# votnhan/VN_celeb_face_recognition

Hardware: AMD Instinct MI355X
Metric: embeddings/sec @ bs=256 (InceptionResnetV1, 160x160) (higher is better)
Workload: dtype bf16

## Files before the change

vn_celeb_face_recognition_amd/csrc/engine.h:

```cpp
#pragma once
#include <hip/hip_runtime.h>
#include <stdint.h>

#include <string>
#include <unordered_map>
#include <vector>

#include "../../include/vnface.h"
#include "kernels.h"

namespace vnf {

void set_error(const std::string& msg);
int fail(int code, const std::string& msg);
const char* last_error_cstr();

#define VNF_HIP(expr)                                                                         \
  do {                                                                                        \
    hipError_t _e = (expr);                                                                   \
    if (_e != hipSuccess)                                                                     \
      return ::vnf::fail(VNF_E_HIP, std::string(#expr) + ": " + hipGetErrorString(_e));       \
  } while (0)

enum class HandleKind { Encoder = 1, Mlp, Mtcnn, MlpTrainer, Retina, HeadTrainer, ConvProbe, Gallery };

struct HandleBase {
  const HandleKind kind;
  explicit HandleBase(HandleKind k) : kind(k) {}
  int device = 0;
  std::vector<void*> allocs;
  virtual ~HandleBase();
  void* dalloc(size_t bytes);
  void* upload(const void* host, size_t bytes);
};

template <class T>
T* handle_cast(vnf_handle h) {
  HandleBase* b = reinterpret_cast<HandleBase*>(h);
  return (b && b->kind == T::KIND) ? static_cast<T*>(b) : nullptr;
}

template <class T>
T* handle_cast_base(vnf_handle h) {
  HandleBase* b = reinterpret_cast<HandleBase*>(h);
  if (b)
    for (HandleKind k : T::KINDS)
      if (b->kind == k) return static_cast<T*>(b);
  return nullptr;
}

struct WeightMap {
  std::unordered_map<std::string, const vnf_tensor_desc*> m;
  std::string missing;
  WeightMap(const vnf_tensor_desc* w, int n);
  const float* get(const std::string& name, int64_t numel);
  bool has(const std::string& name) const { return m.count(name) != 0; }
};

void convert_to(int dtype, const float* src, void* dst, size_t n);

struct Buf {
  int H, W, C;
  size_t elems_per_image() const { return (size_t)H * W * C; }
  char* ptr = nullptr;
};

struct ConvLayer {
  std::string name;
  int x_buf, x_coff, cin;
  int H, W, Ho, Wo, KH, KW, sh, sw, ph, pw;
  void* w = nullptr;
  float* bias = nullptr;
  float* slope = nullptr;
  int4* ktab = nullptr;
  int K, Kpad, cout, cout_pad, ncls = 1;
  int nseg = 0;
  struct { int c0, c1, buf, coff; } seg[4];
  int res_buf = -1, res_coff = 0;
  int act = ACT_NONE, out_f32 = 0;
  int cfg = -1;
  double macs_alg = 0, macs_exec = 0;
};

struct Op {
  enum Kind { PACK, CONV, MAXPOOL, AVGPOOL, L2NORM, COPYOUT, STEM1, DWCONV, UPADD, RSTEM, DWPW, HEADS, SE } kind;
  int src = -1;
  int dst = -1, dst_coff = 0;
  int layer = -1;
  int res = -1;
  PoolWindow window = {0, 0, false};
  int frame_h = 0, frame_w = 0;
  int n_cls = 0, n_proj = 0, proj_col = 0;

  static Op pack(int dst) { Op o{PACK}; o.dst = dst; return o; }
  static Op conv(int layer) { Op o{CONV}; o.layer = layer; return o; }
  static Op stem1(int layer, int dst) { Op o{STEM1}; o.layer = layer; o.dst = dst; return o; }
  static Op maxpool(int src, int dst, int dst_coff, PoolWindow w = {3, 0, false}) {
    Op o{MAXPOOL}; o.src = src; o.dst = dst; o.dst_coff = dst_coff; o.window = w; return o;
  }
  static Op maxpool_ceil(int src, int dst, int k) { return maxpool(src, dst, 0, {k, 0, true}); }
  static Op maxpool_pad1(int src, int dst) { return maxpool(src, dst, 0, {3, 1, false}); }
  static Op avgpool(int src, int dst) { Op o{AVGPOOL}; o.src = src; o.dst = dst; return o; }
  static Op l2norm() { return Op{L2NORM}; }
  static Op copyout() { return Op{COPYOUT}; }
  static Op dwconv(int layer) { Op o{DWCONV}; o.layer = layer; return o; }
  static Op dwpw(int layer) { Op o{DWPW}; o.layer = layer; return o; }
  static Op upadd(int src, int dst) { Op o{UPADD}; o.src = src; o.dst = dst; return o; }
  static Op rstem(int frame_h, int frame_w, int dst) { Op o{RSTEM}; o.frame_h = frame_h; o.frame_w = frame_w; o.dst = dst; return o; }
  static Op se(int layer, int src, int res, int dst) { Op o{SE}; o.layer = layer; o.src = src; o.res = res; o.dst = dst; return o; }
  static Op heads(int n_cls, int n_proj, int proj_col) { Op o{HEADS}; o.n_cls = n_cls; o.n_proj = n_proj; o.proj_col = proj_col; return o; }
};

struct DwLayer {
  int x_buf, o_buf, C, stride;
  float *w = nullptr, *bias = nullptr;
  float slope = 0.f;
};

struct DwPwLayer {
  int x_buf, o_buf, cin, cout, stride;
  float *dw = nullptr, *dbias = nullptr, *pw = nullptr, *pbias = nullptr;
  float slope = 0.f;
  std::string name;
};

struct SeLayer {
  std::string name;
  int C, part_buf;
  float *w1 = nullptr, *b1 = nullptr, *w2 = nullptr, *b2 = nullptr;
  float slope_se = 0.f, slope_out = 0.f;
};

struct Group { int first, last, chunk; };

struct FusedStack {
  enum class Kind { StemMid, Block35, Block17, Block8 } kind = Kind::Block17;
  std::string label;
  int first = 0, last = 0;
  int in_buf = -1, out_buf = -1;
  int nblocks = 0;
  int conv0 = 0;
  void* wstream = nullptr;
  float* bias = nullptr;
  void* wtail = nullptr;
  bool active = false;
  bool stack = false;
  double macs_alg = 0;
  int ext_last = 0, ext_conv = -1, ext_out_buf = -1;
  bool ext = false;
  int end() const { return ext ? ext_last : last; }
};

struct Tap { int buf, coff, C; };

struct EncoderEnv {
  int fuse = 95, direct_stem = 1, stem1a_mfma = 2, retina_fuse = 3, ws_persist = 1;
  int stem_chunk = 0, ir100_chunk1 = 0, ir100_chunk2 = 0;
  int autotune = 1, force_cfg = -2, tune_lanes = 0, autotune_log = 0;
  bool tune_final = true;
  std::string tune_cache;
  static EncoderEnv read();
};

struct RunExtra {
  float* out2 = nullptr;
  const uint8_t* prep_src = nullptr;
  int prep_s = 0;
};

constexpr int ARCH_MLP = -1, ARCH_RNET = -2, ARCH_ONET = -3, ARCH_RETINA = -5;

struct Encoder : HandleBase {
  static constexpr HandleKind KIND = HandleKind::Encoder;
  Encoder() : HandleBase(KIND) {}
  ~Encoder() override;
  int arch, dtype, max_batch, in_size;
  std::vector<Buf> bufs;
  std::vector<ConvLayer> convs;
  std::vector<DwLayer> dws;
  std::vector<DwPwLayer> dwpws;
  std::vector<SeLayer> ses;
  float *rstem_wa = nullptr, *rstem_bias = nullptr;
  std::vector<Op> ops;
  std::vector<Group> groups;
  std::vector<FusedStack> fused;
  std::vector<int> fused_at;
  int prepare_fused();
  int launch_fused(const FusedStack& f, int n0, int nn, hipStream_t s);
  std::unordered_map<std::string, Tap> taps;
  bool buf_materialised(int buf) const;
  float* emb_raw = nullptr;
  int emb_ld = 512;
  int n_cls = 0, n_proj = 0;
  float* cls_buf = nullptr;
  double macs_alg = 0, macs_exec = 0;
  Encoder* head = nullptr;
  int head_classes = 0, head_in = -1, head_logit = -1;
  float* head_emb = nullptr;
  hipEvent_t head_done = nullptr;

  int add_buf(int H, int W, int C);
  char* at(int buf, int n0, int coff = 0) const {
    return bufs[buf].ptr + ((size_t)n0 * bufs[buf].elems_per_image() + coff) * dtype_size(dtype);
  }
  float* at_f32(int buf, int n0) const { return (float*)at(buf, n0); }
  int finalize();
  int autotune();
  ConvArgs conv_args(const ConvLayer& L, int n0, int nn) const;
  int run(const void* x, int n, int x_dtype, float* out, hipStream_t s, std::string* report = nullptr,
          const RunExtra* extra = nullptr);
  int run_range(const void* x, int i0, int i1, int x_dtype, float* out, hipStream_t s, std::string* report, const RunExtra* extra);
  int write_report(std::vector<hipEvent_t>& prof_ev, const std::vector<int>& prof_op, int n, hipStream_t s, std::string* report) const;
  float* stem_wt = nullptr;
  int n_ctx = 1, next_ctx = 0;
  std::vector<std::vector<char*>> ctx_bufs;
  std::vector<float*> ctx_emb;
  std::vector<hipEvent_t> ctx_ev;
  int select_ctx(hipStream_t s, int* used);
  int max_streams = 4;
  bool tune_dirty = true;
  int tune_lanes = 1;
  int tune_batch = 0;
  const EncoderEnv env = EncoderEnv::read();
  hipStream_t side[4] = {nullptr, nullptr, nullptr, nullptr};
  hipEvent_t join_ev[4] = {nullptr, nullptr, nullptr, nullptr}, fork_ev = nullptr;
};

const char* fused_label(const FusedStack& f);
const char* fused_detail(const FusedStack& f);

int build_irv1(Encoder& e, WeightMap& wm);
int build_ir100(Encoder& e, WeightMap& wm);
int build_seir101(Encoder& e, WeightMap& wm);
int build_rn50_2b(Encoder& e, WeightMap& wm, int num_classes, int num_projections);
int build_retina_mnet(Encoder& e, WeightMap& wm, int H, int W, int head_bufs[3]);
struct NetBufs { int crops, pooled1, pooled2, heads; };
int build_rnet(Encoder& e, WeightMap& wm, bool mid, NetBufs& nb);
int build_onet(Encoder& e, WeightMap& wm, bool mid, NetBufs& nb);

}
```

vn_celeb_face_recognition_amd/csrc/fused.cpp:

```cpp
#include "engine.h"
#include "block35.h"
#include "block8.h"
#include "stem_mid.h"
#include "trunk17.h"

#include <cstring>

namespace vnf {

using Kind = FusedStack::Kind;

namespace {

hipError_t copy_bias(float* dst, const ConvLayer& L) { return hipMemcpy(dst, L.bias, (size_t)L.cout * 4, hipMemcpyDeviceToDevice); }

int prepare_stem_mid(Encoder& e, FusedStack& f) {
  if (!(e.env.fuse & 4)) return VNF_OK;
  const ConvLayer& c2a = e.convs[f.conv0];
  const ConvLayer& c2b = e.convs[f.conv0 + 1];
  if (c2a.cout != 32 || c2a.K != 288 || c2b.cout != 64 || c2b.K != 288 || c2a.ncls != 1 || c2b.ncls != 1)
    return fail(VNF_E_INVALID, "fused stem: unexpected layer shapes");
  bool ext_ok = false;
  if ((e.env.fuse & 8) && f.ext_conv >= 0) {
    const ConvLayer& c3b = e.convs[f.ext_conv];
    ext_ok = c3b.cout == 80 && c3b.K == 64 && c3b.KH == 1 && c3b.ncls == 1 && c3b.nseg == 1 && c3b.res_buf < 0 && c3b.act == ACT_RELU &&
             e.bufs[f.ext_out_buf].C == 80;
  }
  if (e.dtype == F16P && !ext_ok) return VNF_OK;
  StemMidPack pk;
  pk.w[0] = c2a.w; pk.kpad[0] = c2a.Kpad;
  pk.w[1] = c2b.w; pk.kpad[1] = c2b.Kpad;
  f.wstream = e.dalloc(stem_mid_wfrag_bytes(e.dtype));
  f.bias = (float*)e.dalloc(SM_BIAS * 4);
  if (!f.wstream || !f.bias) return VNF_E_HIP;
  VNF_HIP(copy_bias(f.bias, c2a));
  VNF_HIP(copy_bias(f.bias + 32, c2b));
  VNF_HIP(stem_mid_repack(pk, e.dtype, f.wstream, 0));
  VNF_HIP(hipDeviceSynchronize());
  f.macs_alg = c2a.macs_alg + c2b.macs_alg;
  f.active = true;
  f.ext = ext_ok;
  if (ext_ok) f.macs_alg += e.convs[f.ext_conv].macs_alg;
  return VNF_OK;
}

int prepare_block35(Encoder& e, FusedStack& f) {
  if (!(e.env.fuse & 2)) return VNF_OK;
  static const int rows[5] = {96, 32, 32, 32, 256}, ks[5] = {256, 288, 288, 288, 96}, boff[5] = {0, 96, 128, 160, 192};
  const size_t wimg_bytes = block35_wimg_bytes(e.dtype);
  f.wstream = e.dalloc((size_t)f.nblocks * wimg_bytes);
  f.bias = (float*)e.dalloc((size_t)f.nblocks * B35_BIAS * 4);
  if (!f.wstream || !f.bias) return VNF_E_HIP;
  for (int b = 0; b < f.nblocks; ++b) {
    Block35Pack pk;
    float* bias = f.bias + (size_t)b * B35_BIAS;
    pk.bias = bias;
    for (int c = 0; c < 5; ++c) {
      const ConvLayer& L = e.convs[f.conv0 + 5 * b + c];
      if (L.cout != rows[c] || L.K != ks[c] || L.ncls != 1) return fail(VNF_E_INVALID, "fused Block35: unexpected layer shapes");
      pk.w[c] = L.w;
      pk.kpad[c] = L.Kpad;
      VNF_HIP(copy_bias(bias + boff[c], L));
      f.macs_alg += L.macs_alg;
    }
    VNF_HIP(block35_repack(pk, e.dtype, (char*)f.wstream + (size_t)b * wimg_bytes, 0));
  }
  VNF_HIP(hipDeviceSynchronize());
  f.active = true;
  f.stack = (e.env.fuse & 16) && e.dtype != F16P;
  f.ext = false;
  if (f.stack && (e.env.fuse & 32) && f.ext_conv >= 0) {
    const ConvLayer& t = e.convs[f.ext_conv];
    const ConvLayer& last_up = e.convs[f.conv0 + 5 * (f.nblocks - 1) + 4];
    const bool ok = t.KH == 1 && t.KW == 1 && t.K == 256 && t.cout == 192 && t.ncls == 1 && t.nseg == 1 && t.res_buf < 0 &&
                    t.act == ACT_RELU && !t.out_f32 && t.x_buf == last_up.seg[0].buf && t.x_coff == 0 &&
                    t.seg[0].buf == f.ext_out_buf && t.seg[0].coff == 0 && e.bufs[f.ext_out_buf].C == 192;
    if (ok) {
      f.wtail = e.dalloc(B35_TAIL_BYTES);
      if (!f.wtail) return VNF_E_HIP;
      VNF_HIP(block35_tail_repack(t.w, t.Kpad, t.bias, f.wtail, 0));
      VNF_HIP(hipDeviceSynchronize());
      f.ext = true;
      f.macs_alg += t.macs_alg;
    }
  }
  return VNF_OK;
}

int prepare_block8(Encoder& e, FusedStack& f) {
  if (!(e.env.fuse & 64) || e.dtype == F16P) return VNF_OK;
  const ConvLayer& red = e.convs[f.conv0];
  const ConvLayer& c13 = e.convs[f.conv0 + 1];
  const ConvLayer& c31 = e.convs[f.conv0 + 2];
  const std::vector<Buf>& bufs = e.bufs;
  auto plain = [](const ConvLayer& L, int cout, int K) {
    return L.cout == cout && L.K == K && L.Kpad == K && L.ncls == 1 && L.res_buf < 0 && L.act == ACT_RELU && !L.out_f32 &&
           L.sh == 1 && L.sw == 1 && L.H == 3 && L.W == 3 && L.Ho == 3 && L.Wo == 3;
  };
  const bool ok =
      plain(red, 384, 1792) && plain(c13, 192, 576) && plain(c31, 192, 576) && f.last - f.first == 3 &&
      red.KH == 1 && red.KW == 1 && red.x_buf == f.in_buf && red.x_coff == 0 && bufs[f.in_buf].C == 1792 && red.nseg == 2 &&
      red.seg[0].c0 == 0 && red.seg[0].c1 == 192 && red.seg[0].buf == f.out_buf && red.seg[0].coff == 0 &&
      red.seg[1].c0 == 192 && red.seg[1].c1 == 384 && red.seg[1].coff == 0 &&
      c13.KH == 1 && c13.KW == 3 && c13.ph == 0 && c13.pw == 1 && c13.x_buf == red.seg[1].buf && c13.x_coff == 0 &&
      c13.nseg == 1 && c13.seg[0].coff == 0 &&
      c31.KH == 3 && c31.KW == 1 && c31.ph == 1 && c31.pw == 0 && c31.x_buf == c13.seg[0].buf && c31.x_coff == 0 &&
      c31.nseg == 1 && c31.seg[0].buf == f.out_buf && c31.seg[0].coff == 192 && bufs[f.out_buf].C == 384;
  if (!ok) return fail(VNF_E_INVALID, "fused Block8 chain: unexpected layer shapes");
  Block8Pack pk;
  pk.w[0] = red.w; pk.kpad[0] = red.Kpad;
  pk.w[1] = c13.w; pk.kpad[1] = c13.Kpad;
  pk.w[2] = c31.w; pk.kpad[2] = c31.Kpad;
  f.wstream = e.dalloc(block8_stream_bytes());
  f.bias = (float*)e.dalloc(B8_BIAS * 4);
  if (!f.wstream || !f.bias) return VNF_E_HIP;
  VNF_HIP(copy_bias(f.bias, red));
  VNF_HIP(copy_bias(f.bias + 384, c13));
  VNF_HIP(copy_bias(f.bias + 576, c31));
  VNF_HIP(block8_repack(pk, f.wstream, 0));
  VNF_HIP(hipDeviceSynchronize());
  f.macs_alg = red.macs_alg + c13.macs_alg + c31.macs_alg;
  f.active = true;
  return VNF_OK;
}

int prepare_block17(Encoder& e, FusedStack& f) {
  if (!(e.env.fuse & 1)) return VNF_OK;
  Trunk17Pack pk;
  memset(&pk, 0, sizeof pk);
  pk.nblocks = f.nblocks;
  static const int rows[4] = {256, 128, 128, 896}, ks[4] = {896, 896, 896, 256}, boff[4] = {0, 256, 384, 512};
  for (int b = 0; b < f.nblocks; ++b)
    for (int c = 0; c < 4; ++c) {
      const ConvLayer& L = e.convs[f.conv0 + 4 * b + c];
      if (L.cout != rows[c] || L.K != ks[c] || L.Kpad != ks[c] || L.ncls != 1)
        return fail(VNF_E_INVALID, "fused Block17 stack: unexpected layer shapes");
      pk.w[b][c] = L.w;
      pk.kpad[c] = L.Kpad;
      f.macs_alg += L.macs_alg;
    }
  f.wstream = e.dalloc(trunk17_stream_bytes(f.nblocks, e.dtype));
  f.bias = (float*)e.dalloc((size_t)f.nblocks * T17_BIAS * 4);
  if (!f.wstream || !f.bias) return VNF_E_HIP;
  for (int b = 0; b < f.nblocks; ++b)
    for (int c = 0; c < 4; ++c) VNF_HIP(copy_bias(f.bias + (size_t)b * T17_BIAS + boff[c], e.convs[f.conv0 + 4 * b + c]));
  VNF_HIP(trunk17_repack(pk, e.dtype, f.wstream, 0));
  VNF_HIP(hipDeviceSynchronize());
  f.active = true;
  return VNF_OK;
}

}

int Encoder::prepare_fused() {
  for (FusedStack& f : fused) {
    f.active = false;
    if (!env.fuse || (dtype != BF16 && dtype != F16 && dtype != F16P) || f.nblocks < 1 || f.nblocks > T17_MAX_BLOCKS) continue;
    int rc = VNF_OK;
    switch (f.kind) {
      case Kind::StemMid: rc = prepare_stem_mid(*this, f); break;
      case Kind::Block35: rc = prepare_block35(*this, f); break;
      case Kind::Block17: rc = prepare_block17(*this, f); break;
      case Kind::Block8: rc = prepare_block8(*this, f); break;
    }
    if (rc != VNF_OK) return rc;
  }
  return VNF_OK;
}

bool Encoder::buf_materialised(int buf) const {
  for (const FusedStack& f : fused) {
    if (!f.active) continue;
    bool written = false;
    for (int oi = f.first; oi < f.end(); ++oi) {
      const Op& op = ops[oi];
      if (op.kind == Op::CONV) {
        const ConvLayer& L = convs[op.layer];
        for (int i = 0; i < L.nseg; ++i) written |= L.seg[i].buf == buf;
      } else if (op.kind == Op::MAXPOOL) {
        written |= op.dst == buf;
      }
    }
    if (!written) continue;
    bool produced = false;
    switch (f.kind) {
      case Kind::StemMid: produced = buf == (f.ext ? f.ext_out_buf : f.out_buf); break;
      case Kind::Block35:
        for (int b = 0; b < f.nblocks; ++b) produced |= convs[f.conv0 + 5 * b + 4].seg[0].buf == buf;
        produced |= f.ext && buf == f.ext_out_buf;
        break;
      case Kind::Block17: produced = buf == f.out_buf; break;
      case Kind::Block8: produced = buf == f.out_buf; break;
    }
    if (!produced) return false;
  }
  return true;
}

int Encoder::launch_fused(const FusedStack& f, int n0, int nn, hipStream_t s) {
  hipError_t err = hipSuccess;
  const char* what = "";
  switch (f.kind) {
    case Kind::StemMid: {
      const int out = f.ext ? f.ext_out_buf : f.out_buf;
      StemMidArgs sa;
      sa.x = at(f.in_buf, n0); sa.ldx = bufs[f.in_buf].C;
      sa.y = at(out, n0); sa.ldy = bufs[out].C;
      sa.n = nn;
      sa.wfrag = f.wstream; sa.bias = f.bias;
      sa.w3b = nullptr; sa.b3b = nullptr; sa.k3b_pad = 0;
      if (f.ext) {
        const ConvLayer& c3b = convs[f.ext_conv];
        sa.w3b = c3b.w; sa.b3b = c3b.bias; sa.k3b_pad = c3b.Kpad;
      }
      what = "fused stem";
      err = launch_stem_mid(sa, dtype, s);
      break;
    }
    case Kind::Block35:
      if (f.stack) {
        const int in = convs[f.conv0 + 4].res_buf;
        const int out = convs[f.conv0 + 5 * (f.nblocks - 1) + 4].seg[0].buf;
        Block35StackArgs ba;
        ba.x = at(in, n0); ba.ldx = bufs[in].C;
        ba.y = at(out, n0); ba.ldy = bufs[out].C;
        ba.n = nn; ba.nblocks = f.nblocks;
        ba.wimg = f.wstream;
        if (f.ext) {
          ba.wtail = f.wtail;
          ba.ytail = at(f.ext_out_buf, n0);
          ba.ldyt = bufs[f.ext_out_buf].C;
        }
        what = "fused Block35 stack";
        err = launch_block35_stack(ba, dtype, s);
        break;
      }
      what = "fused Block35";
      for (int b = 0; b < f.nblocks && err == hipSuccess; ++b) {
        const ConvLayer& up = convs[f.conv0 + 5 * b + 4];
        Block35Args ba;
        ba.x = at(up.res_buf, n0); ba.ldx = bufs[up.res_buf].C;
        ba.y = at(up.seg[0].buf, n0); ba.ldy = bufs[up.seg[0].buf].C;
        ba.n = nn;
        ba.wimg = (const char*)f.wstream + (size_t)b * block35_wimg_bytes(dtype);
        ba.zero = conv_zero_page();
        err = launch_block35(ba, dtype, s);
      }
      break;
    case Kind::Block17: {
      Trunk17Args ta;
      ta.x = at(f.in_buf, n0); ta.ldx = bufs[f.in_buf].C;
      ta.y = at(f.out_buf, n0); ta.ldy = bufs[f.out_buf].C;
      ta.n = nn; ta.nblocks = f.nblocks;
      ta.wstream = f.wstream; ta.bias = f.bias;
      what = "fused Block17 stack";
      err = launch_trunk17(ta, dtype, s);
      break;
    }
    case Kind::Block8: {
      Block8Args ba;
      ba.x = at(f.in_buf, n0); ba.ldx = bufs[f.in_buf].C;
      ba.y = at(f.out_buf, n0); ba.ldy = bufs[f.out_buf].C;
      ba.n = nn;
      ba.wstream = f.wstream; ba.bias = f.bias;
      what = "fused Block8 chain";
      err = launch_block8(ba, dtype, s);
      break;
    }
  }
  return err == hipSuccess ? VNF_OK : fail(VNF_E_HIP, std::string(what) + ": " + hipGetErrorString(err));
}

const char* fused_label(const FusedStack& f) {
  if (f.kind == Kind::StemMid) return f.ext ? "conv2d_2a+2b+maxpool_3a+3b" : "conv2d_2a+2b+maxpool_3a";
  if (f.kind == Kind::Block8) return f.label.c_str();
  return f.kind == Kind::Block35 ? "repeat_1 (fused blocks)" : "repeat_2 (persistent trunk)";
}

const char* fused_detail(const FusedStack& f) {
  if (f.kind == Kind::StemMid) return "rolling rows, one launch, one workgroup per image";
  if (f.kind == Kind::Block17) return "10 x Block17 in one launch, one workgroup per image";
  if (f.kind == Kind::Block8) return "one launch, G = 3 images per workgroup, weights streamed to registers";
  if (!f.stack) return "5 x Block35, one launch per block, one workgroup per image";
  return f.ext ? "5 x Block35 + mixed_6a.branch1.0 in one launch, x in registers"
               : "5 x Block35 in one launch, x in registers, one workgroup per image";
}

}
```

vn_celeb_face_recognition_amd/csrc/plan_irv1.cpp:

```cpp
#include "plan.h"

namespace vnf {

static bool basic_piece(WeightMap& wm, const std::string& p, int cin, int cout, int kh, int kw, Piece& out) {
  return fill_piece(wm, out, p + ".conv.weight", cout, cin * kh * kw, Epilogue::batchnorm(p + ".bn", 1e-3f));
}

int build_irv1(Encoder& e, WeightMap& wm) {
  e.in_size = 160;
  const int b_in = e.add_buf(160, 160, 8);
  const int b_1a = e.add_buf(79, 79, 32), b_2a = e.add_buf(77, 77, 32), b_2b = e.add_buf(77, 77, 64);
  const int b_3a = e.add_buf(38, 38, 64), b_3b = e.add_buf(38, 38, 80), b_4a = e.add_buf(36, 36, 192);
  const int x35[3] = {e.add_buf(17, 17, 256), e.add_buf(17, 17, 256), e.add_buf(17, 17, 256)};
  const int t35a = e.add_buf(17, 17, 64), t35b = e.add_buf(17, 17, 32), cat35 = e.add_buf(17, 17, 96);
  const int m6a = e.add_buf(17, 17, 192), m6b = e.add_buf(17, 17, 192);
  const int x17[3] = {e.add_buf(8, 8, 896), e.add_buf(8, 8, 896), e.add_buf(8, 8, 896)};
  const int t17a = e.add_buf(8, 8, 128), t17b = e.add_buf(8, 8, 128), cat17 = e.add_buf(8, 8, 256);
  const int m7a = e.add_buf(8, 8, 768), m7b = e.add_buf(8, 8, 256);
  const int x8[3] = {e.add_buf(3, 3, 1792), e.add_buf(3, 3, 1792), e.add_buf(3, 3, 1792)};
  const int t8a = e.add_buf(3, 3, 192), t8b = e.add_buf(3, 3, 192), cat8 = e.add_buf(3, 3, 384);
  const int pool = e.add_buf(1, 1, 1792);

  e.ops.push_back(Op::pack(b_in));

  auto simple = [&](const std::string& name, int xb, int xoff, int cin, int cin_pad, int cout, int kh, int kw, int st,
                    int ph, int pw, int ob, int ooff) -> int {
    ConvSpec s;
    s.name = name; s.x_buf = xb; s.x_coff = xoff; s.cin = cin; s.cin_pad = cin_pad;
    s.KH = kh; s.KW = kw; s.sh = s.sw = st; s.ph = ph; s.pw = pw;
    NEED(single_piece(wm, s, name + ".conv.weight", cout, ob, ooff, Epilogue::batchnorm(name + ".bn", 1e-3f)));
    return add_conv(e, s);
  };
  auto fused1x1 = [&](const std::string& name, std::vector<std::string> prefixes, int xb, int cin, int cout_each,
                      std::vector<SegSpec> segs) -> int {
    ConvSpec s;
    s.name = name; s.x_buf = xb; s.cin = s.cin_pad = cin;
    s.pieces.resize(prefixes.size());
    for (size_t i = 0; i < prefixes.size(); ++i)
      NEED(basic_piece(wm, prefixes[i], cin, cout_each, 1, 1, s.pieces[i]));
    s.segs = segs;
    return add_conv(e, s);
  };
  auto up = [&](const std::string& p, int cat, int cin, int cout, float scale, int xin, int xout, bool relu) -> int {
    ConvSpec s;
    s.name = p + ".conv2d"; s.x_buf = cat; s.cin = s.cin_pad = cin;
    NEED(single_piece(wm, s, p + ".conv2d.weight", cout, xout, 0, Epilogue::biased(p + ".conv2d.bias")));
    Piece& pc = s.pieces[0];
    pc.scale.assign(cout, scale);
    for (int i = 0; i < cout; ++i) pc.bias[i] = pc.bias[i] * scale;
    s.res_buf = xin;
    s.act = relu ? ACT_RELU : ACT_NONE;
    return add_conv(e, s);
  };

  TRY(simple("conv2d_1a", b_in, 0, 3, 8, 32, 3, 3, 2, 0, 0, b_1a, 0));
  {
    const int direct = e.env.direct_stem;
    Piece pc;
    if (direct && basic_piece(wm, "conv2d_1a", 3, 32, 3, 3, pc)) {
      std::vector<float> wt(27 * 32 + 32);
      for (int co = 0; co < 32; ++co) {
        for (int k = 0; k < 27; ++k) wt[k * 32 + co] = pc.w[co * 27 + k] * pc.scale[co];
        wt[27 * 32 + co] = pc.bias[co];
      }
      e.stem_wt = (float*)e.upload(wt.data(), wt.size() * 4);
      if (!e.stem_wt) return VNF_E_HIP;
      e.ops.resize(e.ops.size() - 2);
      e.ops.push_back(Op::stem1((int)e.convs.size() - 1, b_1a));
    }
  }
  {
    FusedStack f;
    f.kind = FusedStack::Kind::StemMid;
    f.first = (int)e.ops.size(); f.conv0 = (int)e.convs.size();
    f.in_buf = b_1a; f.out_buf = b_3a; f.nblocks = 1;
    TRY(simple("conv2d_2a", b_1a, 0, 32, 32, 32, 3, 3, 1, 0, 0, b_2a, 0));
    TRY(simple("conv2d_2b", b_2a, 0, 32, 32, 64, 3, 3, 1, 1, 1, b_2b, 0));
    e.ops.push_back(Op::maxpool(b_2b, b_3a, 0));
    f.last = (int)e.ops.size();
    TRY(simple("conv2d_3b", b_3a, 0, 64, 64, 80, 1, 1, 1, 0, 0, b_3b, 0));
    f.ext_last = (int)e.ops.size(); f.ext_conv = (int)e.convs.size() - 1; f.ext_out_buf = b_3b;
    e.fused.push_back(f);
  }
  TRY(simple("conv2d_4a", b_3b, 0, 80, 80, 192, 3, 3, 1, 0, 0, b_4a, 0));
  TRY(simple("conv2d_4b", b_4a, 0, 192, 192, 256, 3, 3, 2, 0, 0, x35[0], 0));
  const int stem_end = (int)e.ops.size();
  e.taps["conv2d_1a"] = {b_1a, 0, 32}; e.taps["conv2d_2a"] = {b_2a, 0, 32}; e.taps["conv2d_2b"] = {b_2b, 0, 64};
  e.taps["maxpool_3a"] = {b_3a, 0, 64}; e.taps["conv2d_3b"] = {b_3b, 0, 80}; e.taps["conv2d_4a"] = {b_4a, 0, 192};
  e.taps["conv2d_4b"] = {x35[0], 0, 256};

  int cur = 0;
  const int r1_first_op = (int)e.ops.size(), r1_first_conv = (int)e.convs.size();
  for (int i = 0; i < 5; ++i) {
    const std::string p = "repeat_1." + std::to_string(i);
    const int X = x35[cur], Y = x35[cur == 1 ? 2 : 1];
    TRY(fused1x1(p + ".reduce", {p + ".branch0", p + ".branch1.0", p + ".branch2.0"}, X, 256, 32,
                 {{0, 32, cat35, 0}, {32, 96, t35a, 0}}));
    TRY(simple(p + ".branch1.1", t35a, 0, 32, 32, 32, 3, 3, 1, 1, 1, cat35, 32));
    TRY(simple(p + ".branch2.1", t35a, 32, 32, 32, 32, 3, 3, 1, 1, 1, t35b, 0));
    TRY(simple(p + ".branch2.2", t35b, 0, 32, 32, 32, 3, 3, 1, 1, 1, cat35, 64));
    TRY(up(p, cat35, 96, 256, 0.17f, X, Y, true));
    cur = (cur == 1 ? 2 : 1);
  }
  e.taps["repeat_1"] = {x35[cur], 0, 256};
  {
    FusedStack f;
    f.kind = FusedStack::Kind::Block35;
    f.first = r1_first_op; f.last = (int)e.ops.size();
    f.nblocks = 5; f.conv0 = r1_first_conv;
    TRY(simple("mixed_6a.branch1.0", x35[cur], 0, 256, 256, 192, 1, 1, 1, 0, 0, m6a, 0));
    f.ext_last = (int)e.ops.size(); f.ext_conv = (int)e.convs.size() - 1; f.ext_out_buf = m6a;
    e.fused.push_back(f);
  }
  {
    const int X = x35[cur], O = x17[0];
    TRY(simple("mixed_6a.branch0", X, 0, 256, 256, 384, 3, 3, 2, 0, 0, O, 0));
    TRY(simple("mixed_6a.branch1.1", m6a, 0, 192, 192, 192, 3, 3, 1, 1, 1, m6b, 0));
    TRY(simple("mixed_6a.branch1.2", m6b, 0, 192, 192, 256, 3, 3, 2, 0, 0, O, 384));
    e.ops.push_back(Op::maxpool(X, O, 640));
  }
  e.taps["mixed_6a"] = {x17[0], 0, 896};
  cur = 0;
  const int r2_first_op = (int)e.ops.size(), r2_first_conv = (int)e.convs.size();
  for (int i = 0; i < 10; ++i) {
    const std::string p = "repeat_2." + std::to_string(i);
    const int X = x17[cur], Y = x17[cur == 1 ? 2 : 1];
    TRY(fused1x1(p + ".reduce", {p + ".branch0", p + ".branch1.0"}, X, 896, 128,
                 {{0, 128, cat17, 0}, {128, 256, t17a, 0}}));
    TRY(simple(p + ".branch1.1", t17a, 0, 128, 128, 128, 1, 7, 1, 0, 3, t17b, 0));
    TRY(simple(p + ".branch1.2", t17b, 0, 128, 128, 128, 7, 1, 1, 3, 0, cat17, 128));
    TRY(up(p, cat17, 256, 896, 0.10f, X, Y, true));
    cur = (cur == 1 ? 2 : 1);
  }
  e.taps["repeat_2"] = {x17[cur], 0, 896};
  {
    FusedStack f;
    f.kind = FusedStack::Kind::Block17;
    f.first = r2_first_op; f.last = (int)e.ops.size();
    f.in_buf = x17[0]; f.out_buf = x17[cur];
    f.nblocks = 10; f.conv0 = r2_first_conv;
    e.fused.push_back(f);
  }
  {
    const int X = x17[cur], O = x8[0];
    TRY(fused1x1("mixed_7a.reduce", {"mixed_7a.branch0.0", "mixed_7a.branch1.0", "mixed_7a.branch2.0"}, X, 896, 256,
                 {{0, 768, m7a, 0}}));
    TRY(simple("mixed_7a.branch0.1", m7a, 0, 256, 256, 384, 3, 3, 2, 0, 0, O, 0));
    TRY(simple("mixed_7a.branch1.1", m7a, 256, 256, 256, 256, 3, 3, 2, 0, 0, O, 384));
    TRY(simple("mixed_7a.branch2.1", m7a, 512, 256, 256, 256, 3, 3, 1, 1, 1, m7b, 0));
    TRY(simple("mixed_7a.branch2.2", m7b, 0, 256, 256, 256, 3, 3, 2, 0, 0, O, 640));
    e.ops.push_back(Op::maxpool(X, O, 896));
  }
  e.taps["mixed_7a"] = {x8[0], 0, 1792};
  cur = 0;
  for (int i = 0; i < 6; ++i) {
    const std::string p = i < 5 ? "repeat_3." + std::to_string(i) : std::string("block8");
    const int X = x8[cur], Y = x8[cur == 1 ? 2 : 1];
    FusedStack f;
    f.kind = FusedStack::Kind::Block8;
    f.label = p + " chain (reduce+1x3+3x1)";
    f.first = (int)e.ops.size(); f.conv0 = (int)e.convs.size();
    f.in_buf = X; f.out_buf = cat8; f.nblocks = 1;
    TRY(fused1x1(p + ".reduce", {p + ".branch0", p + ".branch1.0"}, X, 1792, 192,
                 {{0, 192, cat8, 0}, {192, 384, t8a, 0}}));
    TRY(simple(p + ".branch1.1", t8a, 0, 192, 192, 192, 1, 3, 1, 0, 1, t8b, 0));
    TRY(simple(p + ".branch1.2", t8b, 0, 192, 192, 192, 3, 1, 1, 1, 0, cat8, 192));
    f.last = (int)e.ops.size();
    e.fused.push_back(f);
    TRY(up(p, cat8, 384, 1792, i < 5 ? 0.20f : 1.0f, X, Y, i < 5));
    cur = (cur == 1 ? 2 : 1);
    if (i == 4) e.taps["repeat_3"] = {x8[cur], 0, 1792};
  }
  e.taps["block8"] = {x8[cur], 0, 1792};
  e.ops.push_back(Op::avgpool(x8[cur], pool));
  e.taps["avgpool_1a"] = {pool, 0, 1792};
  {
    ConvSpec s;
    s.name = "last_linear"; s.x_buf = pool; s.cin = s.cin_pad = 1792;
    NEED(single_piece(wm, s, "last_linear.weight", 512, -2, 0, Epilogue::batchnorm("last_bn", 1e-3f)));
    s.act = ACT_NONE; s.out_f32 = 1;
    TRY(add_conv(e, s));
  }
  e.ops.push_back(Op::l2norm());

  const int fuse_mask = e.env.fuse;
  int chunk = ((fuse_mask & 4) && (e.dtype == BF16 || e.dtype == F16 || (e.dtype == F16P && (fuse_mask & 8)))) ? 256 : 128;
  if (e.env.stem_chunk > 0) chunk = e.env.stem_chunk;
  e.groups.push_back({0, stem_end, chunk});
  e.groups.push_back({stem_end, (int)e.ops.size(), 1 << 30});
  return VNF_OK;
}

}
```

Before: 277,000.

## Fuse mixed_6a branch1 conv chain into one LDS-resident kernel

Adds a dedicated kernel that runs mixed_6a's 1x1, 3x3 and strided 3x3 branch1 convolutions in one launch, with one workgroup per image. The image and intermediate activations stay in LDS, and weights are streamed through a register ring buffer. This removes two intermediate global-memory round trips and two launches. The path is gated by a new fuse bit, now on by default, and it steps aside when the Block35 stack has already absorbed branch1.0. Branch0 is moved after the chain in op order. The trade-off is a large LDS footprint per workgroup, which limits occupancy to one workgroup per CU.

Result: faster. 283,300 (median of 6 runs) (+2.3%).

```diff
diff --git a/vn_celeb_face_recognition_amd/csrc/engine.h b/vn_celeb_face_recognition_amd/csrc/engine.h
--- a/vn_celeb_face_recognition_amd/csrc/engine.h
+++ b/vn_celeb_face_recognition_amd/csrc/engine.h
@@ -134,7 +134,7 @@
 struct Group { int first, last, chunk; };
 
 struct FusedStack {
-  enum class Kind { StemMid, Block35, Block17, Block8 } kind = Kind::Block17;
+  enum class Kind { StemMid, Block35, Block17, Block8, Mixed6a } kind = Kind::Block17;
   std::string label;
   int first = 0, last = 0;
   int in_buf = -1, out_buf = -1;
@@ -154,7 +154,7 @@
 struct Tap { int buf, coff, C; };
 
 struct EncoderEnv {
-  int fuse = 95, direct_stem = 1, stem1a_mfma = 2, retina_fuse = 3, ws_persist = 1;
+  int fuse = 223, direct_stem = 1, stem1a_mfma = 2, retina_fuse = 3, ws_persist = 1;
   int stem_chunk = 0, ir100_chunk1 = 0, ir100_chunk2 = 0;
   int autotune = 1, force_cfg = -2, tune_lanes = 0, autotune_log = 0;
   bool tune_final = true;
diff --git a/vn_celeb_face_recognition_amd/csrc/fused.cpp b/vn_celeb_face_recognition_amd/csrc/fused.cpp
--- a/vn_celeb_face_recognition_amd/csrc/fused.cpp
+++ b/vn_celeb_face_recognition_amd/csrc/fused.cpp
@@ -1,6 +1,7 @@
 #include "engine.h"
 #include "block35.h"
 #include "block8.h"
+#include "mixed6a.h"
 #include "stem_mid.h"
 #include "trunk17.h"
 
@@ -124,6 +125,45 @@
   return VNF_OK;
 }
 
+int prepare_mixed6a(Encoder& e, FusedStack& f) {
+  if (!(e.env.fuse & 128) || e.dtype == F16P) return VNF_OK;
+  for (const FusedStack& g : e.fused)
+    if (g.kind == Kind::Block35 && g.active && g.ext && g.ext_conv == f.conv0) return VNF_OK;
+  const ConvLayer& c0 = e.convs[f.conv0];
+  const ConvLayer& c1 = e.convs[f.conv0 + 1];
+  const ConvLayer& c2 = e.convs[f.conv0 + 2];
+  const std::vector<Buf>& bufs = e.bufs;
+  auto plain = [](const ConvLayer& L, int cout, int K, int kh, int st, int pad, int H, int Ho) {
+    return L.cout == cout && L.K == K && L.Kpad == K && L.ncls == 1 && L.nseg == 1 && L.res_buf < 0 && L.act == ACT_RELU &&
+           !L.out_f32 && L.KH == kh && L.KW == kh && L.sh == st && L.sw == st && L.ph == pad && L.pw == pad && L.H == H &&
+           L.W == H && L.Ho == Ho && L.Wo == Ho && L.x_coff == 0 && L.seg[0].c0 == 0 && L.seg[0].c1 == cout;
+  };
+  bool ok = f.last - f.first == 3 && plain(c0, 192, 256, 1, 1, 0, 17, 17) && plain(c1, 192, 1728, 3, 1, 1, 17, 17) &&
+            plain(c2, 256, 1728, 3, 2, 0, 17, 8);
+  for (int i = 0; ok && i < 3; ++i) ok = e.ops[f.first + i].kind == Op::CONV && e.ops[f.first + i].layer == f.conv0 + i;
+  ok = ok && c0.x_buf == f.in_buf && bufs[f.in_buf].H == 17 && bufs[f.in_buf].W == 17 && bufs[f.in_buf].C == 256 &&
+       c0.seg[0].coff == 0 && bufs[c0.seg[0].buf].C == 192 && c1.x_buf == c0.seg[0].buf && c1.cin == 192 &&
+       c1.seg[0].coff == 0 && bufs[c1.seg[0].buf].C == 192 && c2.x_buf == c1.seg[0].buf && c2.cin == 192 &&
+       c2.seg[0].buf == f.out_buf && bufs[f.out_buf].H == 8 && bufs[f.out_buf].W == 8 && c2.seg[0].coff % 8 == 0 &&
+       bufs[f.out_buf].C % 8 == 0 && c2.seg[0].coff + 256 <= bufs[f.out_buf].C;
+  if (!ok) return fail(VNF_E_INVALID, "fused mixed_6a chain: unexpected layer shapes");
+  Mixed6aPack pk;
+  pk.w[0] = c0.w; pk.kpad[0] = c0.Kpad;
+  pk.w[1] = c1.w; pk.kpad[1] = c1.Kpad;
+  pk.w[2] = c2.w; pk.kpad[2] = c2.Kpad;
+  f.wstream = e.dalloc(mixed6a_stream_bytes());
+  f.bias = (float*)e.dalloc(M6_BIAS * 4);
+  if (!f.wstream || !f.bias) return VNF_E_HIP;
+  VNF_HIP(copy_bias(f.bias, c0));
+  VNF_HIP(copy_bias(f.bias + 192, c1));
+  VNF_HIP(copy_bias(f.bias + 384, c2));
+  VNF_HIP(mixed6a_repack(pk, f.wstream, 0));
+  VNF_HIP(hipDeviceSynchronize());
+  f.macs_alg = c0.macs_alg + c1.macs_alg + c2.macs_alg;
+  f.active = true;
+  return VNF_OK;
+}
+
 int prepare_block17(Encoder& e, FusedStack& f) {
   if (!(e.env.fuse & 1)) return VNF_OK;
   Trunk17Pack pk;
@@ -162,6 +202,7 @@
       case Kind::Block35: rc = prepare_block35(*this, f); break;
       case Kind::Block17: rc = prepare_block17(*this, f); break;
       case Kind::Block8: rc = prepare_block8(*this, f); break;
+      case Kind::Mixed6a: rc = prepare_mixed6a(*this, f); break;
     }
     if (rc != VNF_OK) return rc;
   }
@@ -191,6 +232,7 @@
         break;
       case Kind::Block17: produced = buf == f.out_buf; break;
       case Kind::Block8: produced = buf == f.out_buf; break;
+      case Kind::Mixed6a: produced = buf == f.out_buf; break;
     }
     if (!produced) return false;
   }
@@ -267,13 +309,24 @@
       err = launch_block8(ba, dtype, s);
       break;
     }
+    case Kind::Mixed6a: {
+      Mixed6aArgs ma;
+      ma.x = at(f.in_buf, n0); ma.ldx = bufs[f.in_buf].C;
+      ma.y = at(f.out_buf, n0); ma.ldy = bufs[f.out_buf].C;
+      ma.coff = convs[f.conv0 + 2].seg[0].coff;
+      ma.n = nn;
+      ma.wstream = f.wstream; ma.bias = f.bias;
+      what = "fused mixed_6a chain";
+      err = launch_mixed6a(ma, dtype, s);
+      break;
+    }
   }
   return err == hipSuccess ? VNF_OK : fail(VNF_E_HIP, std::string(what) + ": " + hipGetErrorString(err));
 }
 
 const char* fused_label(const FusedStack& f) {
   if (f.kind == Kind::StemMid) return f.ext ? "conv2d_2a+2b+maxpool_3a+3b" : "conv2d_2a+2b+maxpool_3a";
-  if (f.kind == Kind::Block8) return f.label.c_str();
+  if (f.kind == Kind::Block8 || f.kind == Kind::Mixed6a) return f.label.c_str();
   return f.kind == Kind::Block35 ? "repeat_1 (fused blocks)" : "repeat_2 (persistent trunk)";
 }
 
@@ -281,6 +334,7 @@
   if (f.kind == Kind::StemMid) return "rolling rows, one launch, one workgroup per image";
   if (f.kind == Kind::Block17) return "10 x Block17 in one launch, one workgroup per image";
   if (f.kind == Kind::Block8) return "one launch, G = 3 images per workgroup, weights streamed to registers";
+  if (f.kind == Kind::Mixed6a) return "1x1 + 3x3 + 3x3 s2 in one launch, image in LDS, one workgroup per image";
   if (!f.stack) return "5 x Block35, one launch per block, one workgroup per image";
   return f.ext ? "5 x Block35 + mixed_6a.branch1.0 in one launch, x in registers"
                : "5 x Block35 in one launch, x in registers, one workgroup per image";
diff --git a/vn_celeb_face_recognition_amd/csrc/mixed6a.h b/vn_celeb_face_recognition_amd/csrc/mixed6a.h
--- /dev/null
+++ b/vn_celeb_face_recognition_amd/csrc/mixed6a.h
@@ -0,0 +1,26 @@
+#pragma once
+#include <hip/hip_runtime.h>
+#include <stddef.h>
+
+namespace vnf {
+
+constexpr int M6_BIAS = 640;
+
+struct Mixed6aArgs {
+  const void* x;
+  void* y;
+  int ldx, ldy, coff, n;
+  const void* wstream;
+  const float* bias;
+};
+
+struct Mixed6aPack {
+  const void* w[3];
+  int kpad[3];
+};
+
+size_t mixed6a_stream_bytes();
+hipError_t mixed6a_repack(const Mixed6aPack& p, void* out, hipStream_t s);
+hipError_t launch_mixed6a(const Mixed6aArgs& a, int dtype, hipStream_t s);
+
+}
diff --git a/vn_celeb_face_recognition_amd/csrc/mixed6a.hip b/vn_celeb_face_recognition_amd/csrc/mixed6a.hip
--- /dev/null
+++ b/vn_celeb_face_recognition_amd/csrc/mixed6a.hip
@@ -0,0 +1,248 @@
+#include "mixed6a.h"
+#include "fused_device.h"
+
+namespace vnf {
+
+namespace {
+
+constexpr int M6_PX = 289;
+constexpr int M6_ROWS = 296;
+constexpr int M6_RING = 9;
+constexpr int M6_KS1 = 8;
+constexpr int M6_KS3 = 54;
+constexpr int M6_F1 = 3 * M6_KS1;
+constexpr int M6_F2 = 3 * M6_KS3;
+constexpr int M6_F3 = 2 * M6_KS3;
+constexpr int M6_FRAGS = M6_F1 + M6_F2 + M6_F3;
+constexpr int M6_SLOT = M6_FRAGS + M6_RING;
+constexpr int M6_STREAM_FRAGS = 8 * M6_SLOT;
+constexpr int KT_BYTES = M6_ROWS * 128;
+constexpr int OFF_X = 0;
+constexpr int OFF_A = 0;
+constexpr int OFF_OUT = 3 * KT_BYTES;
+constexpr int OFF_ZERO = 4 * KT_BYTES;
+constexpr int OFF_REACH = 3 * KT_BYTES + 320 * 128;
+constexpr int OFF_BIAS = OFF_REACH;
+constexpr int M6_LDS = OFF_BIAS + M6_BIAS * 4;
+static_assert(M6_ROWS % 8 == 0 && M6_ROWS >= M6_PX, "a tile is whole 8-row LDS-DMA pieces");
+static_assert(4 * 64 * 128 <= KT_BYTES, "the output tile fits X's last K tile");
+static_assert(OFF_ZERO + 256 <= OFF_REACH, "the zero chunk lies inside the allocation");
+static_assert(M6_LDS <= 160 * 1024, "one workgroup's LDS");
+static_assert(M6_F1 % M6_RING == 6 && 18 % M6_RING == 0 && (M6_F1 + M6_F2) % M6_RING == 6 && 36 % M6_RING == 0,
+              "the ring slot of a step must not depend on the tap");
+
+template <typename T>
+__device__ __forceinline__ uint2 bias_relu_round(const f32x4_t& acc, const f32x4_t& bias) {
+  f32x4_t v;
+#pragma unroll
+  for (int e = 0; e < 4; ++e) v[e] = fmaxf(acc[e] + bias[e], 0.f);
+  return pack4<T>(v);
+}
+
+}
+
+template <typename T>
+__global__ __launch_bounds__(512) void mixed6a_chain_kernel(const Mixed6aArgs a) {
+  extern __shared__ __attribute__((aligned(16))) char smem[];
+  const int tid = threadIdx.x, lane = tid & 63;
+  const int wave = __builtin_amdgcn_readfirstlane(tid >> 6);
+  const int frow = lane & 15, fgrp = lane >> 4;
+  const int cg = wave & 3, ph = wave >> 2;
+  const int img = blockIdx.x;
+  const unsigned lds0 = lds_dma_base(smem);
+
+  const uint4* wp = reinterpret_cast<const uint4*>(a.wstream) + (size_t)wave * M6_SLOT * 64 + lane;
+  uint4 wq[M6_RING];
+  ring_prime(wq, wp);
+
+  {
+    const char* src = (const char*)a.x + (size_t)img * M6_PX * a.ldx * 2;
+    const int r = lane >> 3, slot = lane & 7;
+    constexpr int PIECES = 4 * (M6_ROWS / 8);
+#pragma unroll
+    for (int i = 0; i < (PIECES + 7) / 8; ++i) {
+      const int piece = wave + i * 8;
+      if (piece < PIECES) {
+        const int kt = piece / (M6_ROWS / 8), rg = piece - kt * (M6_ROWS / 8);
+        const int p = min(rg * 8 + r, M6_PX - 1);
+        glds16(src + ((size_t)p * a.ldx + kt * 64 + ((slot ^ r) << 3)) * 2, lds0 + OFF_X + kt * KT_BYTES + rg * 1024);
+      }
+    }
+    if (tid < 16) reinterpret_cast<uint4*>(smem + OFF_ZERO)[tid] = uint4{0u, 0u, 0u, 0u};
+    if (tid < M6_BIAS / 4) reinterpret_cast<f32x4_t*>(smem + OFF_BIAS)[tid] = reinterpret_cast<const f32x4_t*>(a.bias)[tid];
+    asm volatile("s_waitcnt vmcnt(0)" ::: "memory");
+  }
+  __syncthreads();
+
+  const int p0 = 160 * ph + frow;
+  const int rowb = p0 * 128;
+  const int rb0 = (fgrp ^ (frow & 7)) << 4, rb1 = rb0 ^ 64;
+  auto quad = [&](int c, int row7) {
+    return (c >> 6) * KT_BYTES + ((((c & 63) >> 3) ^ row7) << 4) + (c & 4) * 2;
+  };
+
+  f32x4_t acc[3][10];
+  auto clear = [&]() {
+#pragma unroll
+    for (int j = 0; j < 3; ++j)
+#pragma unroll
+      for (int i = 0; i < 10; ++i) acc[j][i] = f32x4_t{0.f, 0.f, 0.f, 0.f};
+  };
+  auto store_image = [&](int bias0) {
+#pragma unroll
+    for (int j = 0; j < 3; ++j) {
+      const int c = 16 * (3 * cg + j) + 4 * fgrp;
+      const f32x4_t bv = *reinterpret_cast<const f32x4_t*>(smem + OFF_BIAS + (bias0 + c) * 4);
+      const int qb = OFF_A + quad(c, frow & 7) + rowb;
+#pragma unroll
+      for (int i = 0; i < 10; ++i)
+        if (p0 + 16 * i < M6_PX) *reinterpret_cast<uint2*>(smem + qb + i * 2048) = bias_relu_round<T>(acc[j][i], bv);
+    }
+  };
+
+  clear();
+#pragma unroll
+  for (int ks = 0; ks < M6_KS1; ++ks) {
+    uint4 xf[10];
+#pragma unroll
+    for (int i = 0; i < 10; ++i)
+      xf[i] = *reinterpret_cast<const uint4*>(smem + OFF_X + (ks >> 1) * KT_BYTES + rowb + i * 2048 + ((ks & 1) ? rb1 : rb0));
+#pragma unroll
+    for (int j = 0; j < 3; ++j) {
+      const int s = ks * 3 + j;
+#pragma unroll
+      for (int i = 0; i < 10; ++i) mma_chunk<T>(acc[j][i], wq[s % M6_RING], xf[i]);
+      ring_refill(wq, s, wp);
+    }
+    __builtin_amdgcn_sched_barrier(0);
+  }
+  __syncthreads();
+  store_image(0);
+  __syncthreads();
+
+  {
+    int yx[10];
+#pragma unroll
+    for (int i = 0; i < 10; ++i) {
+      const int p = p0 + 16 * i, y = (p * 241) >> 12;
+      yx[i] = p < M6_PX ? (y << 8) | (p - 17 * y) : 0x4040;
+    }
+    clear();
+#pragma unroll 1
+    for (int tap = 0; tap < 9; ++tap) {
+      const int dy = tap / 3 - 1, dx = tap - 3 * (tap / 3) - 1;
+      int tb[10];
+#pragma unroll
+      for (int i = 0; i < 10; ++i) {
+        const bool ok = (unsigned)((yx[i] >> 8) + dy) < 17u && (unsigned)((yx[i] & 255) + dx) < 17u;
+        const int row = p0 + 16 * i + 17 * dy + dx;
+        tb[i] = ok ? row * 128 + ((fgrp ^ (row & 7)) << 4) : -1;
+      }
+#pragma unroll
+      for (int kk = 0; kk < 6; ++kk) {
+        uint4 xf[10];
+#pragma unroll
+        for (int i = 0; i < 10; ++i) {
+          const int off = OFF_A + (((kk >> 1) * KT_BYTES + tb[i]) ^ ((kk & 1) * 64));
+          xf[i] = *reinterpret_cast<const uint4*>(smem + (tb[i] >= 0 ? off : OFF_ZERO));
+        }
+#pragma unroll
+        for (int j = 0; j < 3; ++j) {
+          const int s = M6_F1 + kk * 3 + j;
+#pragma unroll
+          for (int i = 0; i < 10; ++i) mma_chunk<T>(acc[j][i], wq[s % M6_RING], xf[i]);
+          ring_refill(wq, s, wp);
+        }
+        __builtin_amdgcn_sched_barrier(0);
+      }
+    }
+  }
+  __syncthreads();
+  store_image(192);
+  __syncthreads();
+
+  {
+    f32x4_t o[2][4];
+#pragma unroll
+    for (int j = 0; j < 2; ++j)
+#pragma unroll
+      for (int i = 0; i < 4; ++i) o[j][i] = f32x4_t{0.f, 0.f, 0.f, 0.f};
+    const int in0 = 34 * (frow >> 3) + 2 * (frow & 7);
+#pragma unroll 1
+    for (int dy = 0; dy < 3; ++dy) {
+#pragma unroll
+      for (int dx = 0; dx < 3; ++dx) {
+        int tb[4];
+#pragma unroll
+        for (int i = 0; i < 4; ++i) {
+          const int row = in0 + 68 * i + 17 * dy + dx;
+          tb[i] = row * 128 + ((fgrp ^ (row & 7)) << 4);
+        }
+#pragma unroll
+        for (int kk = 0; kk < 6; ++kk) {
+          uint4 xf[4];
+#pragma unroll
+          for (int i = 0; i < 4; ++i)
+            xf[i] = *reinterpret_cast<const uint4*>(smem + OFF_A + (((kk >> 1) * KT_BYTES + tb[i]) ^ ((kk & 1) * 64)));
+#pragma unroll
+          for (int j = 0; j < 2; ++j) {
+            const int s = M6_F1 + M6_F2 + dx * 12 + kk * 2 + j;
+#pragma unroll
+            for (int i = 0; i < 4; ++i) mma_chunk<T>(o[j][i], wq[s % M6_RING], xf[i]);
+            ring_refill(wq, s, wp);
+          }
+          __builtin_amdgcn_sched_barrier(0);
+        }
+      }
+    }
+#pragma unroll
+    for (int j = 0; j < 2; ++j) {
+      const int c = 32 * wave + 16 * j + 4 * fgrp;
+      const f32x4_t bv = *reinterpret_cast<const f32x4_t*>(smem + OFF_BIAS + (384 + c) * 4);
+      const int qb = OFF_OUT + (c >> 6) * 8192 + frow * 128 + ((((c & 63) >> 3) ^ (frow & 7)) << 4) + (c & 4) * 2;
+#pragma unroll
+      for (int i = 0; i < 4; ++i) *reinterpret_cast<uint2*>(smem + qb + i * 2048) = bias_relu_round<T>(o[j][i], bv);
+    }
+  }
+  __syncthreads();
+  {
+    char* dst = (char*)a.y + ((size_t)img * 64 * a.ldy + a.coff) * 2;
+#pragma unroll
+    for (int it = 0; it < 4; ++it) {
+      const int idx = it * 512 + tid;
+      const int q = idx >> 5, ch = idx & 31;
+      const uint4 v = *reinterpret_cast<const uint4*>(smem + OFF_OUT + (ch >> 3) * 8192 + q * 128 + (((ch & 7) ^ (q & 7)) << 4));
+      *reinterpret_cast<uint4*>(dst + ((size_t)q * a.ldy + ch * 8) * 2) = v;
+    }
+  }
+}
+
+__global__ void mixed6a_repack_kernel(Mixed6aPack p, uint4* __restrict__ out) {
+  const int lane = threadIdx.x & 63;
+  const int frag = blockIdx.x * (blockDim.x >> 6) + (threadIdx.x >> 6);
+  if (frag >= M6_STREAM_FRAGS) return;
+  const int wave = frag / M6_SLOT, s = frag - wave * M6_SLOT, cg = wave & 3;
+  int conv = -1, r0 = 0, k0 = 0;
+  if (s < M6_F1) { conv = 0; r0 = 16 * (3 * cg + s % 3); k0 = 32 * (s / 3); }
+  else if (s < M6_F1 + M6_F2) { const int t = s - M6_F1; conv = 1; r0 = 16 * (3 * cg + t % 3); k0 = 32 * (t / 3); }
+  else if (s < M6_FRAGS) { const int t = s - M6_F1 - M6_F2; conv = 2; r0 = 16 * (2 * wave + t % 2); k0 = 32 * (t / 2); }
+  uint4 v = {0u, 0u, 0u, 0u};
+  if (conv >= 0) v = GatherA16::load(p.w[conv], p.kpad[conv], r0, k0, lane, 0);
+  out[(size_t)frag * 64 + lane] = v;
+}
+
+size_t mixed6a_stream_bytes() { return (size_t)M6_STREAM_FRAGS * 1024; }
+
+hipError_t mixed6a_repack(const Mixed6aPack& p, void* out, hipStream_t s) {
+  hipLaunchKernelGGL(mixed6a_repack_kernel, dim3((M6_STREAM_FRAGS + 3) / 4), dim3(256), 0, s, p, (uint4*)out);
+  return hipGetLastError();
+}
+
+hipError_t launch_mixed6a(const Mixed6aArgs& a, int dtype, hipStream_t s) {
+  if (a.n <= 0) return hipSuccess;
+  if (dtype == BF16) return launch_with_lds<mixed6a_chain_kernel<__bf16>>(a.n, 512, M6_LDS, s, a);
+  if (dtype == F16) return launch_with_lds<mixed6a_chain_kernel<_Float16>>(a.n, 512, M6_LDS, s, a);
+  return hipErrorInvalidValue;
+}
+
+}
diff --git a/vn_celeb_face_recognition_amd/csrc/plan_irv1.cpp b/vn_celeb_face_recognition_amd/csrc/plan_irv1.cpp
--- a/vn_celeb_face_recognition_amd/csrc/plan_irv1.cpp
+++ b/vn_celeb_face_recognition_amd/csrc/plan_irv1.cpp
@@ -114,9 +114,16 @@
   }
   {
     const int X = x35[cur], O = x17[0];
-    TRY(simple("mixed_6a.branch0", X, 0, 256, 256, 384, 3, 3, 2, 0, 0, O, 0));
+    FusedStack f;
+    f.kind = FusedStack::Kind::Mixed6a;
+    f.label = "mixed_6a.branch1.0-1.2 chain";
+    f.first = (int)e.ops.size() - 1; f.conv0 = (int)e.convs.size() - 1;
+    f.in_buf = X; f.out_buf = O; f.nblocks = 1;
     TRY(simple("mixed_6a.branch1.1", m6a, 0, 192, 192, 192, 3, 3, 1, 1, 1, m6b, 0));
     TRY(simple("mixed_6a.branch1.2", m6b, 0, 192, 192, 256, 3, 3, 2, 0, 0, O, 384));
+    f.last = (int)e.ops.size();
+    e.fused.push_back(f);
+    TRY(simple("mixed_6a.branch0", X, 0, 256, 256, 384, 3, 3, 2, 0, 0, O, 0));
     e.ops.push_back(Op::maxpool(X, O, 640));
   }
   e.taps["mixed_6a"] = {x17[0], 0, 896};
```
